# limuhit/360-Image-Compression

Measured on AMD Instinct MI355X. Metric: ERP Mpixels/s enc+dec @512x1024 model-idx 3; bitstream bit-exact vs ref, higher is better.
Workload: dtype f32; 1 GPU; 192/GPU synthetic 512x1024 ERPs, model-idx 3 --ssim seed, latent+importance bitstreams, entropy enc+dec; streams=3, masks=smooth

## Files before the change

### 360-image-compression_amd/csrc/cconv144_kernels.hip

```cpp
#include "common.h"
#include "conv_plan.h"
#include "cconv_tree.h"

#define I144_THREADS 512

template <int C, int HIDDEN>
struct ITerms {
    static constexpr int NIDX = 25 * C;
    static constexpr bool causal(int tap) { return tap / 5 + tap % 5 <= 3 + HIDDEN; }
    static constexpr int nterms(int l) {
        int n = 0;
        for (int i = l; i < NIDX; i += 128) n += causal(i % 25) ? 1 : 0;
        return n;
    }
    static constexpr int term(int l, int t) {
        int n = 0;
        for (int i = l; i < NIDX; i += 128)
            if (causal(i % 25)) { if (n == t) return i; ++n; }
        return -1;
    }
    static constexpr int nquads(int l) { return (nterms(l) + 3) / 4; }
    static constexpr int qbase(int l) {
        int s = 0;
        for (int j = 0; j < l; ++j) s += nquads(j);
        return s;
    }
    static constexpr int NQ = qbase(128);
    static constexpr int nblocks(int c) { int s = 0; for (int a = 0; a < 16; ++a) s += nquads(c + 8 * a); return s; }
    static constexpr int blk_a(int c, int b) { int a = 0; while (b >= nquads(c + 8 * a)) { b -= nquads(c + 8 * a); ++a; } return a; }
    static constexpr int blk_q(int c, int b) { int a = 0; while (b >= nquads(c + 8 * a)) { b -= nquads(c + 8 * a); ++a; } return b; }
    static constexpr int ngroups() { int m = 0; for (int c = 0; c < 8; ++c) { const int g = (nblocks(c) + 3) / 4; m = g > m ? g : m; } return m; }
    static constexpr int NG = ngroups();
};

static inline bool conv144_ok(const lic360_conv_plan *p) {
    return p->ksz == 5 && p->ngroup == 1 && p->C == 144 && p->nout >= 1 && p->nout <= 144 && p->constrain == 6;
}
template <int HIDDEN> static int i144_nq() { return ITerms<144, HIDDEN>::NQ; }
static int conv144_nq(const lic360_conv_plan *p) { (void)p; return i144_nq<1>(); }
static int conv144_otiles(const lic360_conv_plan *p) { return (p->nout + 15) / 16; }

__global__ void k_conv144_pack(const float *__restrict__ weight, const int *__restrict__ src, const int *__restrict__ qmap, float *__restrict__ packed,
                               int nout, int C, int NG, long total) {
    for (long e = (long)blockIdx.x * blockDim.x + threadIdx.x; e < total; e += (long)gridDim.x * blockDim.x) {
        const int jw = (int)(e & 3), l = (int)((e >> 2) & 63), i = l & 15, k = l >> 4;
        const long t = e >> 8;
        const int g = (int)(t % NG), c = (int)((t / NG) & 7), ot = (int)(t / (8 * NG)), o = ot * 16 + i;
        const int Q = qmap[(c * NG + g) * 4 + jw];
        const int s = Q >= 0 ? src[Q * 4 + k] : -1;
        packed[e] = (s >= 0 && o < nout) ? weight[(long)o * C * 25 + s] : 0.0f;
    }
}
template <int HIDDEN>
static void i144_fill_src(int *src, int *qmap) {
    using T = ITerms<144, HIDDEN>;
    int Q = 0;
    for (int l = 0; l < 128; ++l) {
        const int nt = T::nterms(l);
        for (int q = 0; q < T::nquads(l); ++q, ++Q)
            for (int k = 0; k < 4; ++k) src[Q * 4 + k] = 4 * q + k < nt ? T::term(l, 4 * q + k) : -1;
    }
    for (int c = 0; c < 8; ++c)
        for (int b = 0; b < 4 * T::NG; ++b)
            qmap[c * 4 * T::NG + b] = b < T::nblocks(c) ? T::qbase(c + 8 * T::blk_a(c, b)) + T::blk_q(c, b) : -1;
}
LIC360_API int lic360_conv144_supported(const lic360_conv_plan *p) { return p && conv144_ok(p) ? 1 : 0; }
LIC360_API long lic360_conv144_packed_floats(const lic360_conv_plan *p) {
    return p && conv144_ok(p) ? (long)conv144_otiles(p) * 8 * ITerms<144, 1>::NG * 256 : 0;
}
LIC360_API int lic360_conv144_pack(void *stream, const lic360_conv_plan *p, const float *weight, float *packed) {
    ARG_CHECK(p && conv144_ok(p) && weight && packed);
    const int NQ = conv144_nq(p), NG = ITerms<144, 1>::NG, nint = 4 * NQ + 8 * 4 * NG;
    std::vector<int> h(nint);
    i144_fill_src<1>(h.data(), h.data() + 4 * NQ);
    DevBuf<int> d;
    if (d.alloc(nint)) return 1;
    HIP_TRY(hipMemcpyAsync(d, h.data(), sizeof(int) * nint, hipMemcpyHostToDevice, (hipStream_t)stream));
    const long total = lic360_conv144_packed_floats(p);
    hipLaunchKernelGGL(k_conv144_pack, dim3(lic360_blocks(total, 4)), dim3(256), 0, (hipStream_t)stream, weight, d, d + 4 * NQ, packed, p->nout, p->C, NG,
                       total);
    LAUNCH_CHECK();
    HIP_TRY(hipStreamSynchronize((hipStream_t)stream));
    return 0;
}

template <bool DC, int NT>
struct ILay {
    static constexpr int ROWS = DC ? 5 : NT + 4, COLS = DC ? 16 * NT + 4 : 20, QPR = COLS / 4, PLANE = ROWS * COLS, TOFF = DC ? 16 : COLS;
    static constexpr int tap_off(int kh, int kw) { return DC ? (kh + kw) * COLS + kh : kh * COLS + kw; }
};

struct I144Args {
    const float *x, *packed, *bias, *act, *residual;
    float *out;
    int N, H, W, nout, n_ot;
    int grid;
    long xplane, xsample;
    int xpitch;
    long oplane, osample;
    int opitch, ooff;
    int tiles_r, tiles_c;
    int s, th_lo, th_hi, th0;
    int n_seg;
    int og, n_og;
};

#define I144_WAIT0() asm volatile("s_waitcnt vmcnt(0)" ::: "memory")
__device__ __forceinline__ void i144_dma_x4(const float *src, unsigned lds_byte_addr) {
    asm volatile("s_mov_b32 m0, %1\n\ts_nop 0\n\tglobal_load_lds_dwordx4 %0, off" ::"v"(src), "s"(lds_byte_addr) : "memory");
}
__device__ __forceinline__ unsigned i144_lds_addr(const float *p) {
    return (unsigned)(unsigned long)(__attribute__((address_space(3))) const float *)p;
}
__device__ __forceinline__ f32x4 i144_mfma(float a, float b, f32x4 c) { return __builtin_amdgcn_mfma_f32_16x16x4f32(a, b, c, 0, 0, 0); }

#define I144_PFG 2

template <int HIDDEN, bool DC, int NT, int WAVE>
__device__ __forceinline__ void i144_body(const I144Args &a, float *xs, float *comb, const int tid, const int lane) {
    using T = ITerms<144, HIDDEN>;
    using L = ILay<DC, NT>;
    constexpr int C = 144;
    constexpr int XQ = C * L::ROWS * L::QPR;
    constexpr int NDMA = (XQ + 511) / 512;
    const unsigned lds_x = i144_lds_addr(xs);
    int soff[NDMA];
#pragma unroll
    for (int m = 0; m < NDMA; ++m) {
        int e = (WAVE + 8 * m) * 64 + lane;
        if (e >= XQ) e = XQ - 1;
        const int pl = e / (L::ROWS * L::QPR), rem = e - pl * (L::ROWS * L::QPR), row = rem / L::QPR, cq = rem - row * L::QPR;
        soff[m] = (int)(pl * a.xplane) + row * a.xpitch + cq * 4;
    }
    const int kq = lane >> 4, j = lane & 15;
    const int ntasks = DC ? a.N * a.n_og * a.n_seg : a.N * a.tiles_r * a.tiles_c;
    int parity = 0;
    for (int task = blockIdx.x; task < ntasks; task += a.grid) {
        int n, r0 = 0, c0 = 0, ot_lo = 0, ot_hi = a.n_ot, th0 = 0;
        if constexpr (DC) {
            const int per = a.n_og * a.n_seg;
            n = task / per;
            const int rem = task - n * per, seg = rem / a.n_og;
            ot_lo = (rem - seg * a.n_og) * a.og;
            ot_hi = ot_lo + a.og < a.n_ot ? ot_lo + a.og : a.n_ot;
            th0 = a.th0 + seg * (16 * NT);
        } else {
            n = task / (a.tiles_r * a.tiles_c);
            const int rem = task - n * (a.tiles_r * a.tiles_c);
            r0 = (rem / a.tiles_c) * NT;
            c0 = (rem % a.tiles_c) * 16;
        }
        const float *xt = a.x + (long)n * a.xsample + (DC ? (long)(a.s - 4 + I144_R0) * a.xpitch + th0 : (long)r0 * a.xpitch + c0);
        __syncthreads();
        static_for<NDMA>([&](auto mm) {
            constexpr int m = decltype(mm)::value;
            if constexpr ((WAVE + 8 * m) * 64 < XQ) i144_dma_x4(xt + soff[m], lds_x + (unsigned)((WAVE + 8 * m) * 1024));
        });
        I144_WAIT0();
        __syncthreads();
        for (int ot = ot_lo; ot < ot_hi; ++ot) {
            const float *wot = a.packed + ((long)ot * 8 + WAVE) * (T::NG * 256) + lane * 4;
            f32x4 acc[NT][16];
            constexpr int NB = T::nblocks(WAVE), NGW = (NB + 3) / 4, RING = I144_PFG + 1;
            f32x4 aring[RING];
            static_for<(I144_PFG < NGW ? I144_PFG : NGW)>([&](auto gg) {
                constexpr int g = decltype(gg)::value;
                aring[g % RING] = *(const f32x4 *)(wot + g * 256);
            });
            static_for<NB>([&](auto bb) {
                constexpr int b = decltype(bb)::value, aa = T::blk_a(WAVE, b), q = T::blk_q(WAVE, b), l = WAVE + 8 * aa;
                if constexpr (b % 4 == 0 && b / 4 + I144_PFG < NGW) aring[(b / 4 + I144_PFG) % RING] = *(const f32x4 *)(wot + (b / 4 + I144_PFG) * 256);
                const float av = aring[(b / 4) % RING][b % 4];
                constexpr int nt = T::nterms(l);
                auto off_of = [](int k) constexpr {
                    const int t = 4 * q + k < nt ? 4 * q + k : nt - 1, idx = T::term(l, t), tap = idx % 25, gid = idx / 25;
                    return (gid * L::PLANE + L::tap_off(tap / 5, tap % 5)) * 4;
                };
                constexpr int o0 = off_of(0), o1 = off_of(1), o2 = off_of(2), o3 = off_of(3);
                int voff = kq == 1 ? o1 : o0;
                voff = kq == 2 ? o2 : voff;
                voff = kq == 3 ? o3 : voff;
                const float *bp = (const float *)((const char *)xs + voff) + j;
                float bv[NT];
#pragma unroll
                for (int t = 0; t < NT; ++t) bv[t] = bp[t * L::TOFF];
                __builtin_amdgcn_sched_barrier(0);
                const f32x4 zero4 = {0.f, 0.f, 0.f, 0.f};
#pragma unroll
                for (int t = 0; t < NT; ++t) acc[t][aa] = i144_mfma(av, bv[t], q == 0 ? zero4 : acc[t][aa]);
                __builtin_amdgcn_sched_barrier(0);
            });
#pragma unroll
            for (int t = 0; t < NT; ++t) {
                f32x4 lv[8];
#pragma unroll
                for (int i = 0; i < 8; ++i) lv[i] = acc[t][i] + acc[t][i + 8];
#pragma unroll
                for (int i = 0; i < 4; ++i) lv[i] = lv[i] + lv[i + 4];
#pragma unroll
                for (int i = 0; i < 2; ++i) lv[i] = lv[i] + lv[i + 2];
                const f32x4 r = lv[0] + lv[1];
#pragma unroll
                for (int v = 0; v < 4; ++v) comb[((parity * NT + t) * 8 + WAVE) * 256 + v * 64 + lane] = r[v];
            }
            __syncthreads();
            for (int e = tid; e < NT * 256; e += I144_THREADS) {
                const int t = e >> 8, rem = e & 255, v = rem >> 6, ln = rem & 63;
                const float *cb = comb + ((parity * NT + t) * 8) * 256 + v * 64 + ln;
                const float r0_ = cb[0], r1 = cb[256], r2 = cb[512], r3 = cb[768], r4 = cb[1024], r5 = cb[1280], r6 = cb[1536], r7 = cb[1792];
                float sv = ((r0_ + r4) + (r2 + r6)) + ((r1 + r5) + (r3 + r7));
                const int o = ot * 16 + 4 * (ln >> 4) + v, jj = ln & 15;
                bool ok = o < a.nout;
                long oi;
                if constexpr (DC) {
                    const int th = th0 + 16 * t + jj;
                    ok = ok && th >= a.th_lo && th <= a.th_hi;
                    oi = (long)n * a.osample + (long)o * a.oplane + (long)(a.s + I144_R0) * a.opitch + th + I144_C0;
                } else {
                    const int y = r0 + t, xx = c0 + jj;
                    ok = ok && y < a.H && xx < a.W;
                    oi = (long)n * a.osample + (long)o * a.oplane + (long)(y + a.ooff) * a.opitch + xx + a.ooff;
                }
                if (ok) {
                    sv = sv + a.bias[o];
                    if (a.act) sv = DC ? (sv < 0 ? sv * a.act[o] : sv) : (sv > 0 ? sv : sv * a.act[o]);
                    if (a.residual) sv = sv + a.residual[oi];
                    a.out[oi] = sv;
                }
            }
            parity ^= 1;
        }
    }
}

template <int HIDDEN, bool DC, int NT>
__global__ __launch_bounds__(I144_THREADS, 2) void k_cconv144(I144Args a) {
    using L = ILay<DC, NT>;
    __shared__ float xs[144 * L::PLANE + 256];
    __shared__ float comb[2 * NT * 8 * 256];
    const int tid = threadIdx.x, lane = tid & 63;
    const int wave = __builtin_amdgcn_readfirstlane(tid >> 6);
    switch (wave) {
        case 0: i144_body<HIDDEN, DC, NT, 0>(a, xs, comb, tid, lane); break;
        case 1: i144_body<HIDDEN, DC, NT, 1>(a, xs, comb, tid, lane); break;
        case 2: i144_body<HIDDEN, DC, NT, 2>(a, xs, comb, tid, lane); break;
        case 3: i144_body<HIDDEN, DC, NT, 3>(a, xs, comb, tid, lane); break;
        case 4: i144_body<HIDDEN, DC, NT, 4>(a, xs, comb, tid, lane); break;
        case 5: i144_body<HIDDEN, DC, NT, 5>(a, xs, comb, tid, lane); break;
        case 6: i144_body<HIDDEN, DC, NT, 6>(a, xs, comb, tid, lane); break;
        default: i144_body<HIDDEN, DC, NT, 7>(a, xs, comb, tid, lane); break;
    }
}

#define I144_NT_EC 2
#define I144_NT_DC 2

LIC360_API int lic360_ec144_layout(int h, int w, int *hp, int *wp) {
    ARG_CHECK(hp && wp && h > 0 && w > 0);
    *hp = (h + I144_NT_EC - 1) / I144_NT_EC * I144_NT_EC + 4;
    *wp = (w + 15) / 16 * 16 + 4;
    return 0;
}
LIC360_API int lic360_cconv144_ec(void *stream, const lic360_conv_plan *p, const float *x, const float *packed144, const float *bias,
                                  const float *act, const float *residual, float *out, int n, int h, int w, long oplane, int opitch, int ooff) {
    ARG_CHECK(p && conv144_ok(p) && x && packed144 && bias && out && n > 0 && h > 0 && w > 0 && oplane > 0 && opitch > 0 && (ooff == 0 || ooff == 2));
    I144Args a;
    int hp, wp;
    if (lic360_ec144_layout(h, w, &hp, &wp)) return 2;
    a.x = x; a.packed = packed144; a.bias = bias; a.act = act; a.residual = residual; a.out = out;
    a.N = n; a.H = h; a.W = w; a.nout = p->nout; a.n_ot = conv144_otiles(p);
    a.xplane = (long)hp * wp; a.xsample = 144 * a.xplane; a.xpitch = wp;
    a.oplane = oplane; a.osample = (long)p->nout * oplane; a.opitch = opitch; a.ooff = ooff;
    a.tiles_r = (h + I144_NT_EC - 1) / I144_NT_EC; a.tiles_c = (w + 15) / 16;
    a.s = a.th_lo = a.th_hi = a.th0 = 0; a.og = a.n_ot; a.n_og = 1; a.n_seg = 1;
    const long ntasks = (long)n * a.tiles_r * a.tiles_c;
    const dim3 grid((unsigned)(ntasks < 256 ? ntasks : 256));
    a.grid = (int)grid.x;
    hipLaunchKernelGGL((k_cconv144<1, false, I144_NT_EC>), grid, dim3(I144_THREADS), 0, (hipStream_t)stream, a);
    LAUNCH_CHECK();
    return 0;
}

LIC360_API int lic360_dc144_layout(int h, int w, int *rows, int *pitch) {
    ARG_CHECK(rows && pitch && h > 0 && w > 0);
    *rows = h + w - 1 + 2 * I144_R0;
    *pitch = (h + 2 * I144_C0 + 16 * I144_NT_DC + 3) / 4 * 4;
    return 0;
}
LIC360_API int lic360_cconv144_dc_plane(void *stream, const lic360_conv_plan *p, const float *x, const float *packed144, const float *bias,
                                        const float *act, const float *residual, float *out, int n, int h, int w, int s) {
    ARG_CHECK(p && conv144_ok(p) && x && packed144 && bias && out && n > 0 && h > 0 && w > 0);
    if (s < 0 || s >= h + w - 1) return 0;
    I144Args a;
    int rows, pitch;
    if (lic360_dc144_layout(h, w, &rows, &pitch)) return 2;
    a.x = x; a.packed = packed144; a.bias = bias; a.act = act; a.residual = residual; a.out = out;
    a.N = n; a.H = h; a.W = w; a.nout = p->nout; a.n_ot = conv144_otiles(p);
    a.xplane = (long)rows * pitch; a.xsample = 144 * a.xplane; a.xpitch = pitch;
    a.oplane = a.xplane; a.osample = (long)p->nout * a.xplane; a.opitch = pitch; a.ooff = 0;
    a.tiles_r = a.tiles_c = 1;
    a.s = s; a.th_lo = s >= w ? s - w + 1 : 0; a.th_hi = s < h ? s : h - 1; a.th0 = a.th_lo & ~3;
    a.n_seg = (a.th_hi - a.th0) / (16 * I144_NT_DC) + 1;
    a.og = a.n_ot;
    while (a.og > 1 && (long)n * a.n_seg * ((a.n_ot + a.og - 1) / a.og) < 192) --a.og;
    a.n_og = (a.n_ot + a.og - 1) / a.og;
    const long ntasks = (long)n * a.n_og * a.n_seg;
    const dim3 grid((unsigned)(ntasks < 256 ? ntasks : 256));
    a.grid = (int)grid.x;
    hipLaunchKernelGGL((k_cconv144<1, true, I144_NT_DC>), grid, dim3(I144_THREADS), 0, (hipStream_t)stream, a);
    LAUNCH_CHECK();
    return 0;
}
```

### 360-image-compression_amd/csrc/codec_fused.hip

```cpp
#include "common.h"
#include "conv_plan.h"
#include "ac_core.h"
#include "lic360_exact_math.h"
#include "gmm_tables.h"
#include "need.h"
#include <vector>
#include <cstring>
#include <algorithm>
#include <thread>
#include <atomic>
#include <memory>
#include <immintrin.h>

struct AcDevState {
    uint32_t low, high, code;
    int nacc, error, pad;
    long pos;
    unsigned long long acc;
};

struct PlanDeleter { void operator()(lic360_conv_plan *p) const { lic360_conv_plan_destroy(p); } };
using PlanPtr = std::unique_ptr<lic360_conv_plan, PlanDeleter>;
static int make_plan(PlanPtr &out, int channel, int ngroup, int nout, int ksz, int constrain) {
    lic360_conv_plan *p = nullptr;
// ... 1319 lines not shown
        return lic360_cconv144_ec(stream, nw.at(layer), xin, nw.xpack[0][layer], nw.bias[layer], nw.act[layer], res, dst, B, H, W, (long)c->e_hp * c->e_wp, c->e_wp, 2);
    };
    float *y = c->use144 ? c->e_plain : c->e_buf[1];
    if (net_walk(c->e_x0, c->use144 ? c->e_pad : c->e_buf, 3, y, ec)) return 1;
    if (c->nsym == IMP_NSYM_FAST) hipLaunchKernelGGL(k_imp_enc_tables<true>, dim3(lic360_blocks(total, 1)), dim3(64), 0, s, y, levels, c->d_pidx, c->e_rec, B, H, W, c->nsym);
    else hipLaunchKernelGGL(k_imp_enc_tables<false>, dim3(lic360_blocks(total, 1)), dim3(64), 0, s, y, levels, c->d_pidx, c->e_rec, B, H, W, c->nsym);
    LAUNCH_CHECK();
    hipLaunchKernelGGL(k_ac_encode, dim3(B), dim3(128), 0, s, c->e_rec, (long)c->HW, bytes, cap, nbytes, err);
    LAUNCH_CHECK();
    return 0;
}
struct ImpMaskPlaneArgs {
    const float *levels;
    const int *idx;
    int start;
    int len;
    float *out;
    int B;
    int H;
    int W;
    int C;
    int s;
    int cpn;
};
__global__ void k_imp_mask_plane(const ImpMaskPlaneArgs a) {
    const float *__restrict__ levels = a.levels;
    const int *__restrict__ idx = a.idx;
    const int start = a.start;
    const int len = a.len;
    float *__restrict__ out = a.out;
    const int B = a.B;
    const int H = a.H;
    const int W = a.W;
    const int C = a.C;
    const int s = a.s;
    const int cpn = a.cpn;
    const long HW = (long)H * W, total = (long)B * len * C;
    const int Co = C / (s * s), Ho = H * s, Wo = W * s;
    const long e = (long)blockIdx.x * 256 + threadIdx.x;
    if (e < total) {
        const int tc = (int)(e % C), i = (int)((e / C) % len), b = (int)(e / C / len);
        const int th = idx[start + i], tw = idx[start + i + HW];
        const int imp = (int)((double)levels[(long)b * HW + (long)th * W + tw] + 1e-5) * cpn;
        const int pc = tc / (s * s), r = tc % (s * s), ph = th * s + r / s, pw = tw * s + r % s;
        out[(((long)b * Co + pc) * Ho + ph) * Wo + pw] = tc < imp ? 1.0f : 0.0f;
    }
}
static int impcodec_decode_impl(void *stream, lic360_impcodec *c, const uint8_t *bytes, long cap, const int *nbytes, int B,
                                float *levels_out, int *err, float *mask_out, int mask_c, int stride) {
    if (check_ready(c, B)) return 2;
    ARG_CHECK(nbytes && levels_out && err);
    if (check_slot(bytes, cap)) return 2;
    hipStream_t s = (hipStream_t)stream;
    const int H = c->H, W = c->W;
    hipLaunchKernelGGL(k_dec_init, dim3((B + 63) / 64), dim3(64), 0, s, bytes, cap, nbytes, c->d_state, B);
    LAUNCH_CHECK();
    const int *pih = c->h_pidx.data();
    const long SK = (long)c->sk_rows * c->sk_pitch, off0 = (long)c->sk_row0 * c->sk_pitch + c->sk_col0;
    const NetWeights &nw = c->w;
    for (int p = 0; p < c->P; ++p) {
        if (net_walk(c->d_x0, c->d_act, 11, c->d_y, [&](int layer, const float *xin, const float *res, float *dst) -> int {
                if (c->use144 && layer > 0)
                    return lic360_cconv144_dc_plane(stream, nw.at(layer), xin, nw.xpack[0][layer], nw.bias[layer], nw.act[layer], res, dst, B, H, W, p);
                return lic360_cconv_dc_plane_strided(stream, nw.at(layer), xin + off0, nw.packed[layer], nw.bias[layer], nw.act[layer],
                                                     res ? res + off0 : nullptr, dst + off0, B, H, W, 1, c->d_idx, c->d_pidx, pih, p, B,
                                                     SK, c->sk_pitch + 1, c->sk_pitch, SK, c->sk_pitch + 1, c->sk_pitch);
            })) return 1;
        const int start = pih[p], len = pih[p + 1] - pih[p];
        if (len <= 0) continue;
        if (c->nsym == IMP_NSYM_FAST)
            hipLaunchKernelGGL(k_imp_dec_tables<true>, dim3((len + 63) / 64, B), dim3(64), 0, s, ImpDecTablesArgs{c->d_y, c->d_idx, start, len, c->d_tab, c->tab_pitch, H, W, c->nsym,
                               c->sk_rows, c->sk_pitch, c->sk_row0, c->sk_col0});
        else
            hipLaunchKernelGGL(k_imp_dec_tables<false>, dim3((len + 63) / 64, B), dim3(64), 0, s, ImpDecTablesArgs{c->d_y, c->d_idx, start, len, c->d_tab, c->tab_pitch, H, W, c->nsym,
                               c->sk_rows, c->sk_pitch, c->sk_row0, c->sk_col0});
        LAUNCH_CHECK();
        hipLaunchKernelGGL(k_imp_dec_plane<false>, dim3(B), dim3(64), 0, s, ImpDecPlaneArgs{c->d_tab, c->tab_pitch, c->d_idx, start, len, c->d_state, bytes, cap, nbytes,
                           c->d_x0, levels_out, H, W, c->nsym, c->sc, c->sk_rows, c->sk_pitch, c->sk_row0, c->sk_col0});
        LAUNCH_CHECK();
        if (mask_out) {
            const long tot = (long)B * len * mask_c;
            hipLaunchKernelGGL(k_imp_mask_plane, dim3((unsigned)((tot + 255) / 256)), dim3(256), 0, s, ImpMaskPlaneArgs{levels_out, c->d_idx, start, len, mask_out, B, H, W,
                               mask_c, stride, mask_c / (c->nsym - 1)});
            LAUNCH_CHECK();
            HIP_TRY(hipEventRecord(c->plane_ev[p], s));
        }
    }
    hipLaunchKernelGGL(k_collect_err, dim3((B + 63) / 64), dim3(64), 0, s, c->d_state, err, B);
    LAUNCH_CHECK();
    return 0;
}
LIC360_API int lic360_impcodec_decode(void *stream, lic360_impcodec *c, const uint8_t *bytes, long cap, const int *nbytes, int B,
                                      float *levels_out, int *err) {
    return impcodec_decode_impl(stream, c, bytes, cap, nbytes, B, levels_out, err, nullptr, 0, 0);
}
LIC360_API int lic360_impcodec_decode_masked(void *stream, lic360_impcodec *c, const uint8_t *bytes, long cap, const int *nbytes, int B,
                                             float *levels_out, int *err, float *mask_out, int mask_c, int stride, long *generation_out) {
    ARG_CHECK(c && mask_out && generation_out && mask_c > 0 && stride > 0 && mask_c % (stride * stride) == 0 && c->nsym > 1 &&
              mask_c % (c->nsym - 1) == 0 && B > 0 && B <= c->maxB);
    while ((int)c->plane_ev.size() < c->P) {
        HipEvent e;
        if (e.create(hipEventDisableTiming | hipEventDisableSystemFence)) return 1;
        c->plane_ev.push_back(std::move(e));
    }
    const int rc = impcodec_decode_impl(stream, c, bytes, cap, nbytes, B, levels_out, err, mask_out, mask_c, stride);
    c->gate_armed = rc == 0;
    if (rc) return rc;
    c->gate_stride = stride;
    c->gate_B = B;
    c->gate_mask = mask_out;
    *generation_out = ++c->gate_gen;
    return 0;
}

LIC360_API int lic360_codec_decode_gated(void *stream, lic360_codec *c, const uint8_t *bytes, long cap, const int *nbytes,
                                         const float *mask, int B, float *code_out, int *err, lic360_impcodec *map_codec, long generation) {
    ARG_CHECK(map_codec && generation > 0);
    if (!map_codec->gate_armed || map_codec->gate_gen != generation) {
        lic360_set_error("lic360_codec_decode_gated: stale gate (generation %ld, the map codec is at %ld, %s): enqueue "
                         "lic360_impcodec_decode_masked of THIS step first, and use each gate once",
                         generation, map_codec->gate_gen, map_codec->gate_armed ? "armed" : "already consumed");
        return 2;
    }
    if (map_codec->gate_mask != mask) {
        lic360_set_error("lic360_codec_decode_gated: `mask` is not the buffer the masked decode of generation %ld fills", generation);
        return 2;
    }
    if (B > map_codec->gate_B) {
        lic360_set_error("lic360_codec_decode_gated: batch %d, but the masked decode of generation %ld fills the mask of %d images", B, generation, map_codec->gate_B);
        return 2;
    }
    if (const int rc = check_decode(c, bytes, cap, nbytes, mask, B, code_out, err)) return rc;
    map_codec->gate_armed = false;
    return codec_decode_impl(stream, c, bytes, cap, nbytes, mask, B, code_out, err, map_codec->plane_ev.data(), map_codec->P,
                             map_codec->gate_stride);
}

__global__ void k_test_records(const int *__restrict__ tables, int ncode, const int *__restrict__ labels, const float *__restrict__ mask,
                               long n, uint2 *__restrict__ rec) {
    GRID_STRIDE(i, n) {
        uint2 r = make_uint2(0u, 0u);
        if (!mask || !(mask[i] < 0.5f)) {
            const int *T = tables + i * (ncode + 1);
            int sym = labels[i];
            sym = sym < 0 ? 0 : (sym > ncode - 1 ? ncode - 1 : sym);
            r = make_uint2((unsigned)T[sym], (unsigned)T[sym + 1]);
        }
        rec[i] = r;
    }
}
__global__ void k_test_tab8(const int *__restrict__ tables, const float *__restrict__ mask, long start, int len, uint4 *__restrict__ tab, AcDevState *st) {
    const int i = blockIdx.x * blockDim.x + threadIdx.x;
    if (i >= len) return;
    const int *T = tables + (start + i) * 9;
    const bool coded = !mask || !(mask[start + i] < 0.5f);
    if (coded && ((T[1] | T[2] | T[3] | T[4] | T[5] | T[6] | T[7]) & ~0xffff)) atomicOr(&st->error, 64);
    if (coded && T[7] == 0) atomicOr(&st->error, 64);
    uint4 r = make_uint4(0u, 0u, 0u, 0u), r2 = r;
    if (coded) dec_pack8(T, r, r2);
    tab[2 * i] = r;
    tab[2 * i + 1] = r2;
}
__global__ void k_test_tabn(const int *__restrict__ tables, int ncode, long start, int len, int *__restrict__ tab) {
    const int i = blockIdx.x, k = threadIdx.x;
    if (i < len && k <= ncode) tab[(long)i * IMP_TW + k] = tables[(start + i) * (ncode + 1) + k];
}

LIC360_API int lic360_devcoder_encode(void *stream, const int *tables, int ncode, const int *labels, const float *mask, long n,
                                      uint8_t *bytes, long cap, int *nbytes, int *err) {
    ARG_CHECK(ncode >= 1 && n >= 0 && nbytes && err && (n == 0 || (tables && labels)));
    if (check_slot(bytes, cap)) return 2;
    hipStream_t s = (hipStream_t)stream;
    DevBuf<uint2> rec;
    if (rec.alloc((size_t)n)) return 1;
    if (n) {
        hipLaunchKernelGGL(k_test_records, dim3(lic360_blocks(n, 1)), dim3(256), 0, s, tables, ncode, labels, mask, n, rec);
        LAUNCH_CHECK();
    }
    hipLaunchKernelGGL(k_ac_encode, dim3(1), dim3(128), 0, s, rec, n, bytes, cap, nbytes, err);
    LAUNCH_CHECK();
    HIP_TRY(hipStreamSynchronize(s));
    return 0;
}

LIC360_API int lic360_devcoder_decode(void *stream, const int *tables, int ncode, const float *mask, long n, int chunk,
                                      const uint8_t *bytes, long cap, const int *nbytes, float *out, int *err) {
    ARG_CHECK(ncode >= 1 && ncode < IMP_TW && n >= 0 && chunk > 0 && nbytes && out && err && (n == 0 || tables) && (ncode == 8 || !mask));
    if (check_slot(bytes, cap)) return 2;
    hipStream_t s = (hipStream_t)stream;
    DevBuf<AcDevState> st;
    DevBuf<uint4> tab8;
    DevBuf<int> tabn;
    if (st.alloc(1) || tab8.alloc(2 * (size_t)chunk) || tabn.alloc((size_t)chunk * IMP_TW)) return 1;
    hipLaunchKernelGGL(k_dec_init, dim3(1), dim3(64), 0, s, bytes, cap, nbytes, st, 1);
    LAUNCH_CHECK();
    for (long start = 0; start < n; start += chunk) {
        const int len = (int)std::min<long>(chunk, n - start);
        if (ncode == 8) {
            hipLaunchKernelGGL(k_test_tab8, dim3((len + 63) / 64), dim3(64), 0, s, tables, mask, start, len, tab8, st);
            LAUNCH_CHECK();
            hipLaunchKernelGGL(k_dec_plane<true>, dim3(1), dim3(64), 0, s, DecPlaneArgs{tab8, chunk, (const int *)nullptr, (int)start, len, 0, st, bytes, cap, nbytes,
                               (float *)nullptr, out, 0, 1, 1, 0, 0, 0, 0});
        } else {
            hipLaunchKernelGGL(k_test_tabn, dim3(len), dim3(64), 0, s, tables, ncode, start, len, tabn);
            LAUNCH_CHECK();
            hipLaunchKernelGGL(k_imp_dec_plane<true>, dim3(1), dim3(64), 0, s, ImpDecPlaneArgs{tabn, chunk, (const int *)nullptr, (int)start, len, st, bytes, cap, nbytes,
                               (float *)nullptr, out, 0, 0, ncode, 0.0f});
        }
        LAUNCH_CHECK();
    }
    hipLaunchKernelGGL(k_collect_err, dim3(1), dim3(64), 0, s, st, err, 1);
    LAUNCH_CHECK();
    HIP_TRY(hipStreamSynchronize(s));
    return 0;
}

LIC360_API int lic360_codec_profile_enable(lic360_codec *c, int on) {
    ARG_CHECK(c);
    c->prof = on != 0;
    for (int k = 0; k < PROF_NCLS; ++k) c->n_ev[k] = 0;
    return 0;
}
LIC360_API const char *lic360_codec_profile_classes(void) { return PROF_NAMES; }

LIC360_API int lic360_codec_profile_read(lic360_codec *c, int n, double *ms, long *launches) {
    ARG_CHECK(c && ms && launches && n >= PROF_NCLS);
    for (int k = 0; k < PROF_NCLS; ++k) {
        double acc = 0;
        const size_t cnt = c->n_ev[k];
        for (size_t i = 0; i + 1 < cnt; i += 2) {
            HIP_TRY(hipEventSynchronize(c->ev[k][i + 1]));
            float t = 0;
            HIP_TRY(hipEventElapsedTime(&t, c->ev[k][i], c->ev[k][i + 1]));
            acc += t;
        }
        ms[k] = acc;
        launches[k] = (long)(cnt / 2);
        c->n_ev[k] = 0;
    }
    return 0;
}

LIC360_API int lic360_codec_skip_stats(lic360_codec *c, int enable, unsigned long long *out, int *skip_active_out) {
    ARG_CHECK(c);
    if (skip_active_out) *skip_active_out = c->skip ? 1 + (c->dcl.list ? 1 : 0) : 0;
    if (!c->skip) { if (out) memset(out, 0, 2 * NEED_LAYERS * NEED_STAT_G * sizeof(unsigned long long)); return 0; }
    if (enable >= 0) c->stats_on = enable != 0;
    if (out) {
        HIP_TRY(hipDeviceSynchronize());
        HIP_TRY(hipMemcpy(out, c->stats, 2 * NEED_LAYERS * NEED_STAT_G * sizeof(unsigned long long), hipMemcpyDeviceToHost));
        HIP_TRY(hipMemset(c->stats, 0, 2 * NEED_LAYERS * NEED_STAT_G * sizeof(unsigned long long)));
    }
    return 0;
}
__global__ void k_fill_enc(float *buf, long planes, int H, int W, int hp, int wp, int off, float v) {
    GRID_STRIDE(i, planes * H * W) {
        const int x = (int)(i % W), y = (int)((i / W) % H);
        buf[(i / ((long)H * W)) * hp * wp + e_cell(y, x, wp, off)] = v;
    }
}
__global__ void k_fill_dec(float *buf, long planes, int H, int W, int sk_rows, int sk_pitch, int row0, int col0, float v) {
    GRID_STRIDE(i, planes * H * W) {
        const int x = (int)(i % W), y = (int)((i / W) % H);
        buf[(i / ((long)H * W)) * sk_rows * sk_pitch + (long)(y + x + row0) * sk_pitch + y + col0] = v;
    }
}
LIC360_API int lic360_codec_debug_fill(void *stream, lic360_codec *c, float value) {
    ARG_CHECK(c && value == value && value - value == 0.0f);
    hipStream_t s = (hipStream_t)stream;
    const long B = c->maxB, G = c->G;
    for (int i = 0; i < 3; ++i) {
        hipLaunchKernelGGL(k_fill_enc, dim3(lic360_blocks(3 * B * 4 * G * c->HW, 4)), dim3(256), 0, s, c->e_buf[i], 3 * B * 4 * G, c->H, c->W, c->e_hp, c->e_wp, c->e_off, value);
        LAUNCH_CHECK();
    }
    for (int i = 0; i < 11; ++i) {
        hipLaunchKernelGGL(k_fill_dec, dim3(lic360_blocks(3 * B * 4 * G * c->HW, 4)), dim3(256), 0, s, c->d_act[i], 3 * B * 4 * G, c->H, c->W, c->sk_rows, c->sk_pitch, c->sk_row0, c->sk_col0, value);
        LAUNCH_CHECK();
    }
    hipLaunchKernelGGL(k_fill_dec, dim3(lic360_blocks(3 * B * 3 * G * c->HW, 4)), dim3(256), 0, s, c->d_y, 3 * B * 3 * G, c->H, c->W, c->sk_rows, c->sk_pitch, c->sk_row0, c->sk_col0, value);
    LAUNCH_CHECK();
    return 0;
}
LIC360_API int lic360_codec_debug_lists(lic360_codec *c, int which, void *host_out, long bytes, int *cap_out) {
    ARG_CHECK(c && host_out && bytes >= 0 && which >= 0 && which <= 4 && c->skip);
    HIP_TRY(hipDeviceSynchronize());
    const void *src = nullptr;
    long have = 0;
    if (which == 0) { src = c->need; have = (long)c->maxB * NEED_LAYERS * c->HW; }
    else if (which == 1) { src = c->ecl.cnt; have = NEED_LAYERS * 8 * 4L; }
    else if (which == 2) { src = c->ecl.list; have = (long)NEED_LAYERS * 8 * c->ecl.cap * 4; }
    else if (which == 3) { src = c->dcl.cnt; have = c->dcl.list ? (long)NEED_LAYERS * c->P * 8 * 4 : 0; }
    else { src = c->dcl.list; have = c->dcl.list ? (long)NEED_LAYERS * c->P * 8 * c->dcl.cap * 16 : 0; }
    if (cap_out) *cap_out = which <= 2 ? c->ecl.cap : c->dcl.cap;
    ARG_CHECK(src && bytes <= have);
    HIP_TRY(hipMemcpy(host_out, src, (size_t)bytes, hipMemcpyDeviceToHost));
    return 0;
}

LIC360_API const char *lic360_codec_kernel_names(void) {
    return "ec_first=k_cconv16<1, false>;ec_hidden=k_cconv16s+k_cconv16<4, false>;ec_last=k_cconv16<4, true>;"
           "dc_first=k_cconv4v6<1, false, false>+k_cconv4v6t<1>;"
           "dc_hidden=k_cconv4v6l<4>+k_cconv4v6t<4>+k_cconv4v6<4, false, false>+k_cconv4v6<4, false, true>;"
           "dc_last=k_cconv4v6l<4>+k_cconv4v6t<4>+k_cconv4v6<4, false, false>+k_cconv4v6<4, false, true>;"
           "imp_ec=k_cconv144<1, false, 2>;imp_dc=k_cconv144<1, true, 2>";
}
```

Baseline: 60.11 Mpixel/s.

## Rebalance diagonal 144-channel conv work into contiguous units with NT=1 variant

```diff
diff --git a/360-image-compression_amd/csrc/cconv144_kernels.hip b/360-image-compression_amd/csrc/cconv144_kernels.hip
--- a/360-image-compression_amd/csrc/cconv144_kernels.hip
+++ b/360-image-compression_amd/csrc/cconv144_kernels.hip
@@ -102,7 +102,6 @@
     int tiles_r, tiles_c;
     int s, th_lo, th_hi, th0;
     int n_seg;
-    int og, n_og;
 };
 
 #define I144_WAIT0() asm volatile("s_waitcnt vmcnt(0)" ::: "memory")
@@ -113,6 +112,9 @@
     return (unsigned)(unsigned long)(__attribute__((address_space(3))) const float *)p;
 }
 __device__ __forceinline__ f32x4 i144_mfma(float a, float b, f32x4 c) { return __builtin_amdgcn_mfma_f32_16x16x4f32(a, b, c, 0, 0, 0); }
+
+template <bool DC, int NT> struct I144Occ { static constexpr int value = DC && NT == 1 ? 4 : 2; };
+template <bool DC, int NT> struct I144Bpf { static constexpr int value = DC ? (NT == 1 ? 2 : 1) : 0; };
 
 #define I144_PFG 2
 
@@ -132,25 +134,9 @@
         const int pl = e / (L::ROWS * L::QPR), rem = e - pl * (L::ROWS * L::QPR), row = rem / L::QPR, cq = rem - row * L::QPR;
         soff[m] = (int)(pl * a.xplane) + row * a.xpitch + cq * 4;
     }
-    const int kq = lane >> 4, j = lane & 15;
-    const int ntasks = DC ? a.N * a.n_og * a.n_seg : a.N * a.tiles_r * a.tiles_c;
+    const int kq0 = lane >> 4, j = lane & 15;
     int parity = 0;
-    for (int task = blockIdx.x; task < ntasks; task += a.grid) {
-        int n, r0 = 0, c0 = 0, ot_lo = 0, ot_hi = a.n_ot, th0 = 0;
-        if constexpr (DC) {
-            const int per = a.n_og * a.n_seg;
-            n = task / per;
-            const int rem = task - n * per, seg = rem / a.n_og;
-            ot_lo = (rem - seg * a.n_og) * a.og;
-            ot_hi = ot_lo + a.og < a.n_ot ? ot_lo + a.og : a.n_ot;
-            th0 = a.th0 + seg * (16 * NT);
-        } else {
-            n = task / (a.tiles_r * a.tiles_c);
-            const int rem = task - n * (a.tiles_r * a.tiles_c);
-            r0 = (rem / a.tiles_c) * NT;
-            c0 = (rem % a.tiles_c) * 16;
-        }
-        const float *xt = a.x + (long)n * a.xsample + (DC ? (long)(a.s - 4 + I144_R0) * a.xpitch + th0 : (long)r0 * a.xpitch + c0);
+    auto stage = [&](const float *xt) {
         __syncthreads();
         static_for<NDMA>([&](auto mm) {
             constexpr int m = decltype(mm)::value;
@@ -158,83 +144,116 @@
         });
         I144_WAIT0();
         __syncthreads();
-        for (int ot = ot_lo; ot < ot_hi; ++ot) {
-            const float *wot = a.packed + ((long)ot * 8 + WAVE) * (T::NG * 256) + lane * 4;
-            f32x4 acc[NT][16];
-            constexpr int NB = T::nblocks(WAVE), NGW = (NB + 3) / 4, RING = I144_PFG + 1;
-            f32x4 aring[RING];
-            static_for<(I144_PFG < NGW ? I144_PFG : NGW)>([&](auto gg) {
-                constexpr int g = decltype(gg)::value;
-                aring[g % RING] = *(const f32x4 *)(wot + g * 256);
-            });
-            static_for<NB>([&](auto bb) {
-                constexpr int b = decltype(bb)::value, aa = T::blk_a(WAVE, b), q = T::blk_q(WAVE, b), l = WAVE + 8 * aa;
-                if constexpr (b % 4 == 0 && b / 4 + I144_PFG < NGW) aring[(b / 4 + I144_PFG) % RING] = *(const f32x4 *)(wot + (b / 4 + I144_PFG) * 256);
-                const float av = aring[(b / 4) % RING][b % 4];
-                constexpr int nt = T::nterms(l);
-                auto off_of = [](int k) constexpr {
-                    const int t = 4 * q + k < nt ? 4 * q + k : nt - 1, idx = T::term(l, t), tap = idx % 25, gid = idx / 25;
-                    return (gid * L::PLANE + L::tap_off(tap / 5, tap % 5)) * 4;
-                };
-                constexpr int o0 = off_of(0), o1 = off_of(1), o2 = off_of(2), o3 = off_of(3);
-                int voff = kq == 1 ? o1 : o0;
-                voff = kq == 2 ? o2 : voff;
-                voff = kq == 3 ? o3 : voff;
-                const float *bp = (const float *)((const char *)xs + voff) + j;
-                float bv[NT];
-#pragma unroll
-                for (int t = 0; t < NT; ++t) bv[t] = bp[t * L::TOFF];
-                __builtin_amdgcn_sched_barrier(0);
-                const f32x4 zero4 = {0.f, 0.f, 0.f, 0.f};
-#pragma unroll
-                for (int t = 0; t < NT; ++t) acc[t][aa] = i144_mfma(av, bv[t], q == 0 ? zero4 : acc[t][aa]);
-                __builtin_amdgcn_sched_barrier(0);
-            });
-#pragma unroll
-            for (int t = 0; t < NT; ++t) {
-                f32x4 lv[8];
-#pragma unroll
-                for (int i = 0; i < 8; ++i) lv[i] = acc[t][i] + acc[t][i + 8];
-#pragma unroll
-                for (int i = 0; i < 4; ++i) lv[i] = lv[i] + lv[i + 4];
-#pragma unroll
-                for (int i = 0; i < 2; ++i) lv[i] = lv[i] + lv[i + 2];
-                const f32x4 r = lv[0] + lv[1];
-#pragma unroll
-                for (int v = 0; v < 4; ++v) comb[((parity * NT + t) * 8 + WAVE) * 256 + v * 64 + lane] = r[v];
+    };
+    auto run_otile = [&](const int ot, const int n, const int r0, const int c0, const int th0) {
+        const float *wot = a.packed + ((long)ot * 8 + WAVE) * (T::NG * 256) + lane * 4;
+        int kq = kq0;
+        if constexpr (I144Occ<DC, NT>::value > 2) asm volatile("" : "+v"(kq));
+        f32x4 acc[NT][16];
+        constexpr int NB = T::nblocks(WAVE), NGW = (NB + 3) / 4, RING = I144_PFG + 1;
+        f32x4 aring[RING];
+        static_for<(I144_PFG < NGW ? I144_PFG : NGW)>([&](auto gg) {
+            constexpr int g = decltype(gg)::value;
+            aring[g % RING] = *(const f32x4 *)(wot + g * 256);
+        });
+        auto bload = [&](auto bxc, float *dst) {
+            constexpr int bx = decltype(bxc)::value, l = WAVE + 8 * T::blk_a(WAVE, bx), q = T::blk_q(WAVE, bx), nt = T::nterms(l);
+            auto off_of = [](int k) constexpr {
+                const int t = 4 * q + k < nt ? 4 * q + k : nt - 1, idx = T::term(l, t), tap = idx % 25, gid = idx / 25;
+                return (gid * L::PLANE + L::tap_off(tap / 5, tap % 5)) * 4;
+            };
+            constexpr int o0 = off_of(0), o1 = off_of(1), o2 = off_of(2), o3 = off_of(3);
+            int voff = kq == 1 ? o1 : o0;
+            voff = kq == 2 ? o2 : voff;
+            voff = kq == 3 ? o3 : voff;
+            const float *bp = (const float *)((const char *)xs + voff) + j;
+#pragma unroll
+            for (int t = 0; t < NT; ++t) dst[t] = bp[t * L::TOFF];
+        };
+        constexpr int BPF = I144Bpf<DC, NT>::value, BR = BPF + 1;
+        float bring[BR][NT];
+        static_for<(BPF < NB ? BPF : NB)>([&](auto dd) { bload(dd, bring[decltype(dd)::value % BR]); });
+        static_for<NB>([&](auto bb) {
+            constexpr int b = decltype(bb)::value, aa = T::blk_a(WAVE, b), q = T::blk_q(WAVE, b);
+            if constexpr (b % 4 == 0 && b / 4 + I144_PFG < NGW) aring[(b / 4 + I144_PFG) % RING] = *(const f32x4 *)(wot + (b / 4 + I144_PFG) * 256);
+            const float av = aring[(b / 4) % RING][b % 4];
+            if constexpr (BPF == 0) bload(bb, bring[0]);
+            else if constexpr (b + BPF < NB) bload(IC<b + BPF>{}, bring[(b + BPF) % BR]);
+            const float *bv = bring[b % BR];
+            __builtin_amdgcn_sched_barrier(0);
+            const f32x4 zero4 = {0.f, 0.f, 0.f, 0.f};
+#pragma unroll
+            for (int t = 0; t < NT; ++t) acc[t][aa] = i144_mfma(av, bv[t], q == 0 ? zero4 : acc[t][aa]);
+            __builtin_amdgcn_sched_barrier(0);
+        });
+#pragma unroll
+        for (int t = 0; t < NT; ++t) {
+            f32x4 lv[8];
+#pragma unroll
+            for (int i = 0; i < 8; ++i) lv[i] = acc[t][i] + acc[t][i + 8];
+#pragma unroll
+            for (int i = 0; i < 4; ++i) lv[i] = lv[i] + lv[i + 4];
+#pragma unroll
+            for (int i = 0; i < 2; ++i) lv[i] = lv[i] + lv[i + 2];
+            const f32x4 r = lv[0] + lv[1];
+#pragma unroll
+            for (int v = 0; v < 4; ++v) comb[((parity * NT + t) * 8 + WAVE) * 256 + v * 64 + lane] = r[v];
+        }
+        __syncthreads();
+        for (int e = tid; e < NT * 256; e += I144_THREADS) {
+            const int t = e >> 8, rem = e & 255, v = rem >> 6, ln = rem & 63;
+            const float *cb = comb + ((parity * NT + t) * 8) * 256 + v * 64 + ln;
+            const float r0_ = cb[0], r1 = cb[256], r2 = cb[512], r3 = cb[768], r4 = cb[1024], r5 = cb[1280], r6 = cb[1536], r7 = cb[1792];
+            float sv = ((r0_ + r4) + (r2 + r6)) + ((r1 + r5) + (r3 + r7));
+            const int o = ot * 16 + 4 * (ln >> 4) + v, jj = ln & 15;
+            bool ok = o < a.nout;
+            long oi;
+            if constexpr (DC) {
+                const int th = th0 + 16 * t + jj;
+                ok = ok && th >= a.th_lo && th <= a.th_hi;
+                oi = (long)n * a.osample + (long)o * a.oplane + (long)(a.s + I144_R0) * a.opitch + th + I144_C0;
+            } else {
+                const int y = r0 + t, xx = c0 + jj;
+                ok = ok && y < a.H && xx < a.W;
+                oi = (long)n * a.osample + (long)o * a.oplane + (long)(y + a.ooff) * a.opitch + xx + a.ooff;
             }
-            __syncthreads();
-            for (int e = tid; e < NT * 256; e += I144_THREADS) {
-                const int t = e >> 8, rem = e & 255, v = rem >> 6, ln = rem & 63;
-                const float *cb = comb + ((parity * NT + t) * 8) * 256 + v * 64 + ln;
-                const float r0_ = cb[0], r1 = cb[256], r2 = cb[512], r3 = cb[768], r4 = cb[1024], r5 = cb[1280], r6 = cb[1536], r7 = cb[1792];
-                float sv = ((r0_ + r4) + (r2 + r6)) + ((r1 + r5) + (r3 + r7));
-                const int o = ot * 16 + 4 * (ln >> 4) + v, jj = ln & 15;
-                bool ok = o < a.nout;
-                long oi;
-                if constexpr (DC) {
-                    const int th = th0 + 16 * t + jj;
-                    ok = ok && th >= a.th_lo && th <= a.th_hi;
-                    oi = (long)n * a.osample + (long)o * a.oplane + (long)(a.s + I144_R0) * a.opitch + th + I144_C0;
-                } else {
-                    const int y = r0 + t, xx = c0 + jj;
-                    ok = ok && y < a.H && xx < a.W;
-                    oi = (long)n * a.osample + (long)o * a.oplane + (long)(y + a.ooff) * a.opitch + xx + a.ooff;
-                }
-                if (ok) {
-                    sv = sv + a.bias[o];
-                    if (a.act) sv = DC ? (sv < 0 ? sv * a.act[o] : sv) : (sv > 0 ? sv : sv * a.act[o]);
-                    if (a.residual) sv = sv + a.residual[oi];
-                    a.out[oi] = sv;
-                }
+            if (ok) {
+                sv = sv + a.bias[o];
+                if (a.act) sv = DC ? (sv < 0 ? sv * a.act[o] : sv) : (sv > 0 ? sv : sv * a.act[o]);
+                if (a.residual) sv = sv + a.residual[oi];
+                a.out[oi] = sv;
             }
-            parity ^= 1;
         }
+        parity ^= 1;
+    };
+    if constexpr (DC) {
+        const int per = a.n_seg * a.n_ot, U = a.N * per;
+        const int u_lo = (int)((long)blockIdx.x * U / a.grid), u_hi = (int)((long)(blockIdx.x + 1) * U / a.grid);
+        int n = 0, th0 = 0, staged = -1;
+        for (int u = u_lo; u < u_hi; ++u) {
+            const int ms = u / a.n_ot, ot = u - ms * a.n_ot;
+            if (ms != staged) {
+                n = ms / a.n_seg;
+                th0 = a.th0 + (ms - n * a.n_seg) * (16 * NT);
+                stage(a.x + (long)n * a.xsample + (long)(a.s - 4 + I144_R0) * a.xpitch + th0);
+                staged = ms;
+            }
+            run_otile(ot, n, 0, 0, th0);
+        }
+    } else {
+        const int ntasks = a.N * a.tiles_r * a.tiles_c;
+        for (int task = blockIdx.x; task < ntasks; task += a.grid) {
+            const int n = task / (a.tiles_r * a.tiles_c);
+            const int rem = task - n * (a.tiles_r * a.tiles_c);
+            const int r0 = (rem / a.tiles_c) * NT, c0 = (rem % a.tiles_c) * 16;
+            stage(a.x + (long)n * a.xsample + (long)r0 * a.xpitch + c0);
+            for (int ot = 0; ot < a.n_ot; ++ot) run_otile(ot, n, r0, c0, 0);
+        }
     }
 }
 
 template <int HIDDEN, bool DC, int NT>
-__global__ __launch_bounds__(I144_THREADS, 2) void k_cconv144(I144Args a) {
+__global__ __launch_bounds__(I144_THREADS, (I144Occ<DC, NT>::value)) void k_cconv144(I144Args a) {
     using L = ILay<DC, NT>;
     __shared__ float xs[144 * L::PLANE + 256];
     __shared__ float comb[2 * NT * 8 * 256];
@@ -272,7 +291,7 @@
     a.xplane = (long)hp * wp; a.xsample = 144 * a.xplane; a.xpitch = wp;
     a.oplane = oplane; a.osample = (long)p->nout * oplane; a.opitch = opitch; a.ooff = ooff;
     a.tiles_r = (h + I144_NT_EC - 1) / I144_NT_EC; a.tiles_c = (w + 15) / 16;
-    a.s = a.th_lo = a.th_hi = a.th0 = 0; a.og = a.n_ot; a.n_og = 1; a.n_seg = 1;
+    a.s = a.th_lo = a.th_hi = a.th0 = 0; a.n_seg = 1;
     const long ntasks = (long)n * a.tiles_r * a.tiles_c;
     const dim3 grid((unsigned)(ntasks < 256 ? ntasks : 256));
     a.grid = (int)grid.x;
@@ -300,14 +319,14 @@
     a.oplane = a.xplane; a.osample = (long)p->nout * a.xplane; a.opitch = pitch; a.ooff = 0;
     a.tiles_r = a.tiles_c = 1;
     a.s = s; a.th_lo = s >= w ? s - w + 1 : 0; a.th_hi = s < h ? s : h - 1; a.th0 = a.th_lo & ~3;
-    a.n_seg = (a.th_hi - a.th0) / (16 * I144_NT_DC) + 1;
-    a.og = a.n_ot;
-    while (a.og > 1 && (long)n * a.n_seg * ((a.n_ot + a.og - 1) / a.og) < 192) --a.og;
-    a.n_og = (a.n_ot + a.og - 1) / a.og;
-    const long ntasks = (long)n * a.n_og * a.n_seg;
-    const dim3 grid((unsigned)(ntasks < 256 ? ntasks : 256));
+    const bool nt1 = a.th_hi - a.th0 < 16;
+    const int NT = nt1 ? 1 : I144_NT_DC;
+    a.n_seg = (a.th_hi - a.th0) / (16 * NT) + 1;
+    const long units = (long)n * a.n_seg * a.n_ot, slots = nt1 ? 512 : 256;
+    const dim3 grid((unsigned)(units < slots ? units : slots));
     a.grid = (int)grid.x;
-    hipLaunchKernelGGL((k_cconv144<1, true, I144_NT_DC>), grid, dim3(I144_THREADS), 0, (hipStream_t)stream, a);
+    if (nt1) hipLaunchKernelGGL((k_cconv144<1, true, 1>), grid, dim3(I144_THREADS), 0, (hipStream_t)stream, a);
+    else hipLaunchKernelGGL((k_cconv144<1, true, I144_NT_DC>), grid, dim3(I144_THREADS), 0, (hipStream_t)stream, a);
     LAUNCH_CHECK();
     return 0;
 }
diff --git a/360-image-compression_amd/csrc/codec_fused.hip b/360-image-compression_amd/csrc/codec_fused.hip
--- a/360-image-compression_amd/csrc/codec_fused.hip
+++ b/360-image-compression_amd/csrc/codec_fused.hip
@@ -1645,5 +1645,5 @@
            "dc_first=k_cconv4v6<1, false, false>+k_cconv4v6t<1>;"
            "dc_hidden=k_cconv4v6l<4>+k_cconv4v6t<4>+k_cconv4v6<4, false, false>+k_cconv4v6<4, false, true>;"
            "dc_last=k_cconv4v6l<4>+k_cconv4v6t<4>+k_cconv4v6<4, false, false>+k_cconv4v6<4, false, true>;"
-           "imp_ec=k_cconv144<1, false, 2>;imp_dc=k_cconv144<1, true, 2>";
-}
+           "imp_ec=k_cconv144<1, false, 2>;imp_dc=k_cconv144<1, true, 1>+k_cconv144<1, true, 2>";
+}
```

Result: no change. 60.10 Mpixel/s, median of 4 (-0.0%).
